# wdecoster/inquiSTR

Measured on AMD Instinct MI355X. Metric: loci/sec genotyped (inquiSTR call hot path, device-resident batch = L0), higher is better.
Workload: dtype u32/i64; 1 GPU; unphased100k: 100000 loci/GPU x 30 reads x ~200 CIGAR ops, --unphased, device-resident SoA (L0); loci_per_gpu=100000, pairs_per_gpu=3000000, cigar_ops_per_gpu=600007253, minlen=5, support=3, total_loci=100000

## Files before the change

inquistr_amd/csrc/cigar_walk.h:

```cpp
#pragma once
#include <type_traits>

#include "wave_primitives.h"

namespace inq {

typedef unsigned int u32x4 __attribute__((ext_vector_type(4)));

constexpr uint32_t ST_INDEX = 1u, ST_CIGAR_OP = 2u, ST_RANGE = 4u, ST_PHASE = 8u, ST_LOCUS = 16u, ST_HINT = 32u, ST_AUX = 64u,
                   ST_INTERNAL = 128u;

constexpr uint32_t PM_CLIP = 1u, PM_FETCHED = 2u, PM_KEPT = 4u;
constexpr int PM_GRP_SHIFT = 4;
constexpr uint32_t PM_CHOSEN = 64u;

constexpr uint32_t RB_UNMAPPED = 1u, RB_REVERSE = 2u, RB_HAS_HP = 4u, RB_IS_2D = 8u, RB_SA_PANIC = 16u;

constexpr int kQueueCap = 128;

struct Window {
    uint32_t se;
    uint32_t ee;
    uint32_t se1;
    uint32_t width;
    uint32_t minlen;
};

__device__ __forceinline__ Window make_window(uint32_t start, uint32_t end, uint32_t minlen) {
    Window W;
    W.se = start - 10u;
    W.ee = end + 10u;
    W.se1 = W.se + 1u;
    W.width = W.ee >= W.se1 ? W.ee - W.se1 : 0u;
    W.minlen = minlen;
    return W;
}

struct BatchView {
    const uint4 *cigar4;
    const uint4 *reads;
    const uint32_t *pair_read;
    uint64_t n_reads;
    uint64_t n_cigar4;
};

struct QueueEntry {
    u32x4 w;
    uint2 info;
    uint2 pad;
};
struct WaveLds {
    QueueEntry q[kQueueCap];
    unsigned long long acc[64];
    unsigned int flags[64];
    unsigned int endc[64];
};

static_assert(sizeof(WaveLds) == 5120, "a larger WaveLds costs resident workgroups per CU");
static_assert(kQueueCap >= 128, "the list takes the spare words of 128 queue entries");
__device__ __forceinline__ void cont_put(WaveLds &L, uint32_t i, uint32_t cur4, uint32_t rw, uint32_t carry) {
    L.q[i].pad = make_uint2(cur4, rw);
    L.q[64u + i].pad.x = carry;
}
__device__ __forceinline__ void cont_get(const WaveLds &L, int i, uint32_t &cur4, uint32_t &rw, uint32_t &carry) {
    const uint2 r = L.q[i].pad;
    cur4 = r.x, rw = r.y;
    carry = L.q[64 + i].pad.x;
}

struct PairMeta {
    uint32_t off4, nc, pos, misc;
};

__device__ __forceinline__ PairMeta load_pair_meta(const BatchView &b, uint64_t first, int cnt, int lane,
                                                    uint32_t &status, bool &valid) {
    PairMeta m{0u, 0u, 0u, 0u};
    valid = false;
    if (lane < cnt) {
        uint32_t ri = b.pair_read[first + (uint64_t)lane];
        if ((uint64_t)ri < b.n_reads) {
            uint4 r = b.reads[ri];
            uint64_t n4 = ((uint64_t)r.y + 3u) >> 2;
            if (r.y < 0x10000000u && (uint64_t)r.x + n4 <= b.n_cigar4) {
                m.off4 = r.x;
                m.nc = r.y | ((r.w & (RB_IS_2D << 8)) ? 0x80000000u : 0u);
                m.pos = r.z;
                m.misc = r.w;
                valid = true;
            } else {
                status |= ST_INDEX;
            }
        } else {
            status |= ST_INDEX;
        }
    }
    return m;
}

__device__ __forceinline__ uint32_t meta_stage_a(const BatchView &b, uint64_t first, int cnt, int lane) {
    return lane < cnt ? b.pair_read[first + (uint64_t)lane] : 0xffffffffu;
}
__device__ __forceinline__ uint4 meta_stage_b(const BatchView &b, uint32_t ri) {
    return (uint64_t)ri < b.n_reads ? b.reads[ri] : make_uint4(0u, 0xffffffffu, 0u, 0u);
}
__device__ __forceinline__ PairMeta meta_stage_c(const BatchView &b, const uint4 r, int cnt, int lane, uint32_t &status,
                                                  bool &valid) {
    PairMeta m{0u, 0u, 0u, 0u};
    valid = false;
    if (lane < cnt) {
        const uint64_t n4 = ((uint64_t)r.y + 3u) >> 2;
        if (r.y < 0x10000000u && (uint64_t)r.x + n4 <= b.n_cigar4) {
            m.off4 = r.x;
            m.nc = r.y | ((r.w & (RB_IS_2D << 8)) ? 0x80000000u : 0u);
            m.pos = r.z;
            m.misc = r.w;
            valid = true;
        } else {
            status |= ST_INDEX;
        }
    }
    return m;
}

constexpr uint32_t kConsume = 0x18Du;

__device__ __forceinline__ uint32_t ref_advance(uint32_t op, uint32_t len) {
    return len & (uint32_t)__builtin_amdgcn_sbfe((int)kConsume, op, 1u);
}
constexpr uint32_t kConsume32 = kConsume | (kConsume << 16);
__device__ __forceinline__ uint32_t ref_advance_raw(uint32_t w) {
    return (w >> 4) & (uint32_t)__builtin_amdgcn_sbfe((int)kConsume32, w, 1u);
}
constexpr uint32_t kBadOp32 = 0xFE00FE00u;
__device__ __forceinline__ uint32_t bad_ops(const u32x4 w) {
    return (kBadOp32 >> (w.x & 31u)) | (kBadOp32 >> (w.y & 31u)) | (kBadOp32 >> (w.z & 31u)) | (kBadOp32 >> (w.w & 31u));
}
__device__ __forceinline__ void advance4(const u32x4 w, uint32_t &e1, uint32_t &e2, uint32_t &e3, uint32_t &tot) {
    e1 = ref_advance_raw(w.x), e2 = e1 + ref_advance_raw(w.y);
    e3 = e2 + ref_advance_raw(w.z), tot = e3 + ref_advance_raw(w.w);
}

__device__ __forceinline__ void drain_queue(WaveLds &L, uint32_t &qcount, const Window &W, int lane) {
    __builtin_amdgcn_wave_barrier();
    for (uint32_t base = 0; base < qcount; base += 64u) {
        const uint32_t e = base + (uint32_t)lane;
        if (e < qcount) {
            const u32x4 w = L.q[e].w;
            const uint2 info = L.q[e].info;
            const uint32_t rel = info.x;
            const uint32_t slot = info.y & 63u;
            const uint32_t cand_mask = (info.y & 64u) ? 0x06u : 0x16u;
            const uint32_t op0 = w.x & 15u, op1 = w.y & 15u, op2 = w.z & 15u, op3 = w.w & 15u;
            const uint32_t l0 = w.x >> 4, l1 = w.y >> 4, l2 = w.z >> 4, l3 = w.w >> 4;
            const uint32_t e1 = ref_advance(op0, l0), e2 = e1 + ref_advance(op1, l1), e3 = e2 + ref_advance(op2, l2);
            int32_t s = 0;
            uint32_t clip = 0;
#define INQ_OP(op, len, ee_)                                                                              \
    {                                                                                                     \
        const bool hit = ((cand_mask >> (op)) & 1u) && (len) > W.minlen && (rel + (ee_)) < W.width;        \
        const int32_t v = ((op) == 2u) ? -(int32_t)(len) : (int32_t)(len);                                \
        s += hit ? v : 0;                                                                                 \
        clip |= (hit && (op) == 4u) ? 1u : 0u;                                                            \
    }
            INQ_OP(op0, l0, 0u)
            INQ_OP(op1, l1, e1)
            INQ_OP(op2, l2, e2)
            INQ_OP(op3, l3, e3)
#undef INQ_OP
            if (s != 0) atomicAdd(&L.acc[slot], (unsigned long long)(long long)s);
            if (clip) atomicOr(&L.flags[slot], 1u);
        }
    }
    qcount = 0;
    __builtin_amdgcn_wave_barrier();
}

__device__ __forceinline__ bool push_window_lanes(WaveLds &L, uint32_t &qcount, bool inw, const u32x4 w, uint32_t x,
                                                  uint32_t tot, uint32_t info, uint32_t info_mask) {
    const uint64_t mask = ballot64(inw);
    if (mask) {
        QueueEntry *const tail = &L.q[qcount];
        if (inw) {
            const uint32_t idx = __builtin_amdgcn_mbcnt_hi((uint32_t)(mask >> 32), __builtin_amdgcn_mbcnt_lo((uint32_t)mask, 0u));
            tail[idx].w = w;
            tail[idx].info = make_uint2(x - tot, info & info_mask);
        }
        qcount += (uint32_t)__popcll(mask);
    }
    return mask != 0ull && qcount > 64u;
}

template <bool UNPHASED>
__device__ __forceinline__ void read_epilogue(const PairMeta &m, bool valid, int cnt, const Window &W, int lane,
                                              uint32_t end_carry, uint32_t &status, WaveLds &L, int64_t &val,
                                              uint32_t &meta) {
    val = 0;
    meta = 0;
    if (lane < cnt && valid) {
        const uint32_t pos = m.pos;
        const uint32_t mapq = m.misc & 0xffu, bits = (m.misc >> 8) & 0xffu, phase = (m.misc >> 16) & 0xffu;
        uint32_t rlen = end_carry - (pos + 1u);
        if ((bits & RB_UNMAPPED) || rlen == 0u) rlen = 1u;
        const uint32_t rend = pos + rlen;
        const bool fetched = ((int32_t)pos < 0 || pos < W.ee) && rend > W.se;
        bool skip;
        if (UNPHASED)
            skip = W.se < pos || rend < W.ee || mapq <= 10u;
        else
            skip = !(bits & RB_HAS_HP) || (W.se < pos && rend < W.ee) || mapq <= 10u;
        const bool kept = fetched && !skip;
        uint32_t grp = 0u;
        bool bad_phase = false;
        if (!UNPHASED && kept) {
            if (phase > 2u)
                bad_phase = true;
            else
                grp = phase;
        }
        if (bad_phase) status |= ST_PHASE;
        if (kept && (bits & RB_SA_PANIC)) status |= ST_AUX;
        val = (int64_t)L.acc[lane];
        meta = ((L.flags[lane] & 1u) ? PM_CLIP : 0u) | (fetched ? PM_FETCHED : 0u) | (kept ? PM_KEPT : 0u) |
               (grp << PM_GRP_SHIFT);
    }
}

template <bool UNPHASED, int AUX>
__device__ __forceinline__ void walk_pairs_whole(const BatchView &b, const PairMeta &m, bool valid, int cnt,
                                           const Window &W, int lane, uint32_t &status, WaveLds &L, int64_t &val,
                                           uint32_t &meta) {
    L.acc[lane] = 0ull;
    L.flags[lane] = 0u;
    uint32_t qcount = 0;
    uint32_t lane_range = 0, lane_bad = 0;
    uint32_t end_carry = 0;

    const uint4 *cigar4 = b.cigar4;
    asm volatile("" : "+s"(cigar4));
    int hk = 0;
    uint32_t hc = 0, h_nchunks = 1, h_off4 = 0, h_n4 = 0;
    auto head_load = [&]() {
        if (hk < cnt) {
            h_off4 = readlane_u32(m.off4, hk);
            const uint32_t nc = readlane_u32(m.nc, hk) & 0x7fffffffu;
            h_n4 = (nc + 3u) >> 2;
            h_nchunks = max(1u, (nc + 255u) >> 8);
        } else {
            h_off4 = 0;
            h_n4 = 0;
            h_nchunks = 1;
        }
    };
    auto issue = [&]() -> u32x4 {
        const __amdgpu_buffer_rsrc_t rsrc =
            __builtin_amdgcn_make_buffer_rsrc((void *)(cigar4 + h_off4), (short)0, (int)(h_n4 * 16u), 0x00020000);
        const u32x4 v = __builtin_amdgcn_raw_buffer_load_b128(rsrc, (int)((hc * 64u + (uint32_t)lane) * 16u), 0, AUX);
        ++hc;
        if (hc >= h_nchunks) {
            ++hk;
            hc = 0;
            head_load();
        }
        return v;
    };
    head_load();
    u32x4 qa = issue(), qb = issue(), qc = issue(), qd = issue();

    int tk = 0;
    uint32_t tc = 0, t_nchunks = 1, t_nc = 0, t_info = 0, carry = 0;
    auto tail_load = [&]() {
        if (tk < cnt) {
            const uint32_t ncp = readlane_u32(m.nc, tk);
            t_nc = ncp & 0x7fffffffu;
            t_nchunks = max(1u, (t_nc + 255u) >> 8);
            carry = readlane_u32(m.pos, tk) + 1u;
            t_info = (uint32_t)tk | ((ncp >> 31) << 6);
            lane_range |= carry;
        }
    };
    tail_load();

    auto step = [&](const u32x4 w) {
        uint32_t e1, e2, e3, tot;
        advance4(w, e1, e2, e3, tot);
        const uint32_t incl = wave_inclusive_scan_u32(tot);
        lane_bad |= bad_ops(w);
        lane_range |= carry + incl;
        const uint32_t x = (carry - W.se1) + incl;
        if (push_window_lanes(L, qcount, x < W.width + tot, w, x, tot, t_info, ~0u)) drain_queue(L, qcount, W, lane);
        carry += readlane_u32(incl, 63);
        ++tc;
        if (tc >= t_nchunks) {
            end_carry = writelane_u32(end_carry, carry, tk);
            ++tk;
            tc = 0;
            tail_load();
        }
    };

    while (tk < cnt) {
        step(qa);
        qa = issue();
        if (tk < cnt) step(qb);
        qb = issue();
        if (tk < cnt) step(qc);
        qc = issue();
        if (tk < cnt) step(qd);
        qd = issue();
    }
    if (qcount) drain_queue(L, qcount, W, lane);
    if (ballot64((lane_bad & 1u) != 0u)) status |= ST_CIGAR_OP;
    if (ballot64((lane_range >> 31) != 0u)) status |= ST_RANGE;

    read_epilogue<UNPHASED>(m, valid, cnt, W, lane, end_carry, status, L, val, meta);
}

constexpr uint32_t RP_CHECKED = 1u;


constexpr int kHeadLanes = 8;
constexpr int kHeadLines = 4;
__device__ __forceinline__ void head_row_scan_u32(uint32_t x, bool upper, uint32_t &incl, uint32_t &tot) {
    const uint32_t s = row_inclusive_scan_u32(x);
    const uint32_t lower = (uint32_t)__builtin_amdgcn_ds_swizzle((int)s, 0x10 | (0x07 << 5));
    incl = s - (upper ? lower : 0u);
    tot = (uint32_t)__builtin_amdgcn_ds_swizzle((int)incl, 0x18 | (0x07 << 5));
}

struct RowStream {
    uint32_t cur4;
    uint32_t carry;
    uint32_t st;
};
constexpr uint32_t RS_STOP = 128u, RS_LIVE = 256u;
constexpr int RS_LEFT = 9;
constexpr uint32_t kLineMask = 7u;
constexpr uint32_t kRowMaxGroups = 1u << (32 - RS_LEFT);
__host__ __device__ constexpr uint32_t cigar_groups(uint32_t nc) { return (nc + 3u) >> 2; }
static_assert(cigar_groups((1u << 25) - 4u) == kRowMaxGroups - 1u && cigar_groups((1u << 25) - 3u) == kRowMaxGroups,
              "the longest read the row walk takes is 2^25 - 4 ops");
constexpr int RW_SLOT = 23, RW_2D = 30, RW_PROMISED = 31;
static_assert((kRowMaxGroups - 1u) >> RW_SLOT == 0u && (63u << RW_SLOT) >> RW_2D == 0u, "the fields of the row word lie apart");
__device__ __forceinline__ uint32_t rw_pack(uint32_t groups, uint32_t is_2d, bool promised) {
    return groups | (is_2d << RW_2D) | (promised ? 1u << RW_PROMISED : 0u);
}
__device__ __forceinline__ uint32_t rw_groups(uint32_t rw) { return rw & (kRowMaxGroups - 1u); }
__device__ __forceinline__ uint32_t rw_groups_slot0(uint32_t rw) { return rw & ((1u << RW_2D) - 1u); }
__device__ __forceinline__ uint32_t rw_slot(uint32_t rw) { return (rw >> RW_SLOT) & 63u; }
__device__ __forceinline__ uint32_t rw_2d(uint32_t rw) { return (rw >> RW_2D) & 1u; }
__device__ __forceinline__ bool rw_promised(uint32_t rw) { return (rw >> RW_PROMISED) != 0u; }
__device__ __forceinline__ uint32_t row_state(uint32_t groups, uint32_t slot, uint32_t is_2d, bool promised) {
    return (groups << RS_LEFT) | slot | (is_2d << 6) | (promised ? RS_STOP : 0u) | RS_LIVE;
}

template <bool UNPHASED, int AUX>
__device__ __forceinline__ void walk_pairs_rows(const BatchView &b, const PairMeta &m, bool valid, int cnt,
                                                const Window &W, int lane, bool checks, uint32_t &status, WaveLds &L,
                                                int64_t &val, uint32_t &meta) {
    L.acc[lane] = 0ull;
    L.flags[lane] = 0u;
    L.endc[lane] = m.pos + 1u;
    uint32_t qcount = 0;
    uint32_t lane_err = ((m.pos + 1u) >> 31) << 1;
    const uint64_t row_heads = 0x0001000100010001ull;
    const __amdgpu_buffer_rsrc_t rsrc =
        __builtin_amdgcn_make_buffer_rsrc((void *)b.cigar4, (short)0, (int)(uint32_t)(b.n_cigar4 * 16u), 0x00020000);

    const uint32_t d_w = rw_pack(cigar_groups(m.nc & 0x0fffffffu), m.nc >> 31, ((m.misc >> 24) & RP_CHECKED) != 0u);

    const int rl = lane & (kRowLanes - 1);
    const int hl = lane & (kHeadLanes - 1);
    const int hrow = lane >> 3;
    const bool upper = (lane & kHeadLanes) != 0;

    auto issue = [&](const RowStream &S) -> u32x4 {
        const uint32_t g = (S.cur4 & ~kLineMask) + (uint32_t)rl;
        const bool on = g - S.cur4 < (S.st >> RS_LEFT);
        return __builtin_amdgcn_raw_buffer_load_b128(rsrc, (int)(on ? g * 16u : 0xfffffff0u), 0, AUX);
    };
    auto head_issue = [&](const RowStream &S) -> u32x4 {
        return __builtin_amdgcn_raw_buffer_load_b128(rsrc, (int)((uint32_t)hl < (S.st >> RS_LEFT) ? S.cur4 : 0xfffffff0u), 0, AUX);
    };
    auto step = [&](const u32x4 w, RowStream &S, auto lanes, bool last) {
        constexpr uint32_t LANES = decltype(lanes)::value;
        const bool live = S.st != 0u;
        uint32_t e1, e2, e3, tot, incl, rtot;
        advance4(w, e1, e2, e3, tot);
        if (LANES == (uint32_t)kHeadLanes) {
            head_row_scan_u32(tot, upper, incl, rtot);
        } else {
            incl = row_inclusive_scan_u32(tot);
            rtot = row_last(incl);
        }
        if (checks) {
            if (live) {
                lane_err |= bad_ops(w) & 1u;
                lane_err |= ((S.carry + incl) >> 31) << 1;
            }
        }
        const uint32_t x = (S.carry - W.se1) + incl;
        if (push_window_lanes(L, qcount, live && x < W.width + tot, w, x, tot, S.st, 127u)) drain_queue(L, qcount, W, lane);
        S.carry += rtot;
        if (LANES == (uint32_t)kHeadLanes) {
            S.cur4 += 16u * LANES;
            const bool done = last || (S.st >> RS_LEFT) <= LANES || ((S.st & RS_STOP) && S.carry > W.ee);
            if (live && done && hl == 0) L.endc[S.st & 63u] = S.carry;
            S.st = done ? 0u : S.st - (LANES << RS_LEFT);
        } else {
            const uint32_t end4 = (S.cur4 & ~kLineMask) + LANES;
            const uint32_t lim = end4 - S.cur4;
            S.cur4 = end4;
            if (live) {
                if ((S.st >> RS_LEFT) <= lim || ((S.st & RS_STOP) && S.carry > W.ee)) {
                    if (rl == 0) L.endc[S.st & 63u] = S.carry;
                    S.st = 0u;
                } else {
                    S.st -= lim << RS_LEFT;
                }
            }
        }
    };
    using Head = std::integral_constant<uint32_t, (uint32_t)kHeadLanes>;
    using Later = std::integral_constant<uint32_t, (uint32_t)kRowLanes>;

    L.q[lane].pad = make_uint2(m.off4, d_w);
    __builtin_amdgcn_wave_barrier();
    auto assign = [&](RowStream &S, int k0) -> u32x4 {
        S.st = 0u;
        uint32_t voff = 0xfffffff0u;
        if (k0 < cnt) {
            const uint2 d = L.q[k0 + hrow].pad;
            const uint32_t r_w = d.y, skip = d.x & kLineMask;
            S.cur4 = ((d.x & ~kLineMask) + (uint32_t)hl) * 16u;
            S.carry = L.endc[k0 + hrow];
            if (rw_groups_slot0(r_w) != 0u && !(rw_promised(r_w) && S.carry > W.ee)) {
                const uint32_t left = min(rw_groups_slot0(r_w) + skip, (uint32_t)((kHeadLines + 1) * kHeadLanes));
                S.st = row_state(left, (uint32_t)(k0 + hrow), rw_2d(r_w), rw_promised(r_w));
                if ((uint32_t)hl - skip < left - skip) voff = S.cur4;
            }
        }
        return __builtin_amdgcn_raw_buffer_load_b128(rsrc, (int)voff, 0, AUX);
    };
    RowStream sa{0u, 0u, 0u}, sb = sa, sc = sa, sd = sa;
    u32x4 qa, qb, qc, qd;
    for (int k0 = 0; k0 < cnt; k0 += 4 * kHeadLanes) {
        qa = assign(sa, k0);
        qb = assign(sb, k0 + kHeadLanes);
        qc = assign(sc, k0 + 2 * kHeadLanes);
        qd = assign(sd, k0 + 3 * kHeadLanes);
        if (ballot64((sa.st | sb.st | sc.st | sd.st) != 0u)) {
            int line = 0;
            do {
                const bool last = ++line == kHeadLines;
                if (ballot64(sa.st != 0u)) step(qa, sa, Head{}, last);
                qa = head_issue(sa);
                if (ballot64(sb.st != 0u)) step(qb, sb, Head{}, last);
                qb = head_issue(sb);
                if (ballot64(sc.st != 0u)) step(qc, sc, Head{}, last);
                qc = head_issue(sc);
                if (ballot64(sd.st != 0u)) step(qd, sd, Head{}, last);
                qd = head_issue(sd);
            } while (ballot64((sa.st | sb.st | sc.st | sd.st) != 0u));
        }
    }

    __builtin_amdgcn_wave_barrier();
    const uint32_t endc0 = L.endc[lane];
    const uint2 own = L.q[lane].pad;
    const uint32_t groups = rw_groups_slot0(own.y) & (kRowMaxGroups - 1u);
    const bool promised = rw_promised(own.y);
    const uint32_t head_groups = (uint32_t)(kHeadLines * kHeadLanes) - (own.x & kLineMask);
    const bool cont = groups > head_groups && !(promised && endc0 > W.ee);
    const uint64_t cmask = ballot64(cont);
    if (cmask) {
        const int ncont = (int)__popcll(cmask);
        if (cont) {
            const uint32_t i = __builtin_amdgcn_mbcnt_hi((uint32_t)(cmask >> 32), __builtin_amdgcn_mbcnt_lo((uint32_t)cmask, 0u));
            cont_put(L, i, own.x + head_groups, (own.y - head_groups) | ((uint32_t)lane << RW_SLOT), endc0);
        }
        __builtin_amdgcn_wave_barrier();

        int next = 0;
        auto claim = [&](RowStream &S) {
            if (next >= ncont) return;
            const bool idle = S.st == 0u;
            const uint64_t need = ballot64(idle) & row_heads;
            if (need == 0ull) return;
            const int below = (int)__builtin_amdgcn_mbcnt_hi((uint32_t)(need >> 32), __builtin_amdgcn_mbcnt_lo((uint32_t)need, 0u));
            const int k = next + below - ((idle && rl != 0) ? 1 : 0);
            next += (int)__popcll(need);
            if (idle && k < ncont) {
                uint32_t r_w;
                cont_get(L, k, S.cur4, r_w, S.carry);
                S.st = row_state(rw_groups(r_w), rw_slot(r_w), rw_2d(r_w), rw_promised(r_w));
            }
        };
        sa.st = sb.st = sc.st = sd.st = 0u;
        claim(sa);
        qa = issue(sa);
        claim(sb);
        qb = issue(sb);
        claim(sc);
        qc = issue(sc);
        claim(sd);
        qd = issue(sd);
        while (ballot64((sa.st | sb.st | sc.st | sd.st) != 0u)) {
            if (ballot64(sa.st != 0u)) {
                step(qa, sa, Later{}, false);
                claim(sa);
            }
            qa = issue(sa);
            if (ballot64(sb.st != 0u)) {
                step(qb, sb, Later{}, false);
                claim(sb);
            }
            qb = issue(sb);
            if (ballot64(sc.st != 0u)) {
                step(qc, sc, Later{}, false);
                claim(sc);
            }
            qc = issue(sc);
            if (ballot64(sd.st != 0u)) {
                step(qd, sd, Later{}, false);
                claim(sd);
            }
            qd = issue(sd);
        }
    }
    if (qcount) drain_queue(L, qcount, W, lane);
    if (ballot64((lane_err & 1u) != 0u)) status |= ST_CIGAR_OP;
    if (ballot64((lane_err & 2u) != 0u)) status |= ST_RANGE;
    __builtin_amdgcn_wave_barrier();
    read_epilogue<UNPHASED>(m, valid, cnt, W, lane, L.endc[lane], status, L, val, meta);
}

template <bool UNPHASED, int AUX>
__device__ __forceinline__ void walk_pairs(const BatchView &b, const PairMeta &m, bool valid, int cnt,
                                           const Window &W, int lane, uint32_t &status, WaveLds &L, int64_t &val,
                                           uint32_t &meta) {
    const bool checked = lane < cnt && valid && ((m.misc >> 24) & RP_CHECKED) != 0u;
    const bool too_long = lane < cnt && valid && cigar_groups(m.nc & 0x0fffffffu) >= kRowMaxGroups;
    if (ballot64(checked) != 0ull && ballot64(too_long) == 0ull && W.ee >= W.se1 && b.n_cigar4 < (1ull << 28)) {
        const bool checks = ballot64(lane < cnt && valid && !checked) != 0ull;
        walk_pairs_rows<UNPHASED, AUX>(b, m, valid, cnt, W, lane, checks, status, L, val, meta);
    } else {
        walk_pairs_whole<UNPHASED, AUX>(b, m, valid, cnt, W, lane, status, L, val, meta);
    }
}

}
```

Before: 509.3 million loci/s.

## Precompute head row states, specialize checks, and drain queue one wave at a time

Row state and starting carry for each read are now computed once per lane and stored in LDS, so the head assignment only loads them. This removes the per-assign recomputation of groups, skip and the promise check. The head-loop state no longer counts down, and the done/issue tests compare against per-line thresholds instead. The head loop is also instantiated twice on whether checks are on, which removes a runtime branch from every step. The ballot of live lanes is reused for the window push, and drain_queue now handles only the newest 64 entries instead of emptying the whole queue, which shortens each drain but makes drains more frequent and adds code size.

```diff
diff --git a/inquistr_amd/csrc/cigar_walk.h b/inquistr_amd/csrc/cigar_walk.h
--- a/inquistr_amd/csrc/cigar_walk.h
+++ b/inquistr_amd/csrc/cigar_walk.h
@@ -142,7 +142,8 @@
 
 __device__ __forceinline__ void drain_queue(WaveLds &L, uint32_t &qcount, const Window &W, int lane) {
     __builtin_amdgcn_wave_barrier();
-    for (uint32_t base = 0; base < qcount; base += 64u) {
+    const uint32_t base = qcount > 64u ? qcount - 64u : 0u;
+    {
         const uint32_t e = base + (uint32_t)lane;
         if (e < qcount) {
             const u32x4 w = L.q[e].w;
@@ -171,13 +172,12 @@
             if (clip) atomicOr(&L.flags[slot], 1u);
         }
     }
-    qcount = 0;
+    qcount = base;
     __builtin_amdgcn_wave_barrier();
 }
 
-__device__ __forceinline__ bool push_window_lanes(WaveLds &L, uint32_t &qcount, bool inw, const u32x4 w, uint32_t x,
-                                                  uint32_t tot, uint32_t info, uint32_t info_mask) {
-    const uint64_t mask = ballot64(inw);
+__device__ __forceinline__ bool push_window_lanes(WaveLds &L, uint32_t &qcount, uint64_t mask, bool inw, const u32x4 w,
+                                                  uint32_t x, uint32_t tot, uint32_t info, uint32_t info_mask) {
     if (mask) {
         QueueEntry *const tail = &L.q[qcount];
         if (inw) {
@@ -287,7 +287,8 @@
         lane_bad |= bad_ops(w);
         lane_range |= carry + incl;
         const uint32_t x = (carry - W.se1) + incl;
-        if (push_window_lanes(L, qcount, x < W.width + tot, w, x, tot, t_info, ~0u)) drain_queue(L, qcount, W, lane);
+        const bool inw = x < W.width + tot;
+        if (push_window_lanes(L, qcount, ballot64(inw), inw, w, x, tot, t_info, ~0u)) drain_queue(L, qcount, W, lane);
         carry += readlane_u32(incl, 63);
         ++tc;
         if (tc >= t_nchunks) {
@@ -345,7 +346,7 @@
     return groups | (is_2d << RW_2D) | (promised ? 1u << RW_PROMISED : 0u);
 }
 __device__ __forceinline__ uint32_t rw_groups(uint32_t rw) { return rw & (kRowMaxGroups - 1u); }
-__device__ __forceinline__ uint32_t rw_groups_slot0(uint32_t rw) { return rw & ((1u << RW_2D) - 1u); }
+__device__ __forceinline__ uint32_t line_word(uint32_t off4) { return ((off4 & ~kLineMask) << 4) | (off4 & kLineMask); }
 __device__ __forceinline__ uint32_t rw_slot(uint32_t rw) { return (rw >> RW_SLOT) & 63u; }
 __device__ __forceinline__ uint32_t rw_2d(uint32_t rw) { return (rw >> RW_2D) & 1u; }
 __device__ __forceinline__ bool rw_promised(uint32_t rw) { return (rw >> RW_PROMISED) != 0u; }
@@ -378,11 +379,12 @@
         const bool on = g - S.cur4 < (S.st >> RS_LEFT);
         return __builtin_amdgcn_raw_buffer_load_b128(rsrc, (int)(on ? g * 16u : 0xfffffff0u), 0, AUX);
     };
-    auto head_issue = [&](const RowStream &S) -> u32x4 {
-        return __builtin_amdgcn_raw_buffer_load_b128(rsrc, (int)((uint32_t)hl < (S.st >> RS_LEFT) ? S.cur4 : 0xfffffff0u), 0, AUX);
-    };
-    auto step = [&](const u32x4 w, RowStream &S, auto lanes, bool last) {
+    auto head_issue = [&](const RowStream &S, uint32_t next_thr) -> u32x4 {
+        return __builtin_amdgcn_raw_buffer_load_b128(rsrc, (int)(S.st >= next_thr ? S.cur4 : 0xfffffff0u), 0, AUX);
+    };
+    auto step = [&](const u32x4 w, RowStream &S, uint64_t live_mask, auto lanes, auto ck, bool last, uint32_t done_thr) {
         constexpr uint32_t LANES = decltype(lanes)::value;
+        constexpr int CK = decltype(ck)::value;
         const bool live = S.st != 0u;
         uint32_t e1, e2, e3, tot, incl, rtot;
         advance4(w, e1, e2, e3, tot);
@@ -392,26 +394,30 @@
             incl = row_inclusive_scan_u32(tot);
             rtot = row_last(incl);
         }
-        if (checks) {
+        if (CK == 2 ? checks : CK == 1) {
             if (live) {
                 lane_err |= bad_ops(w) & 1u;
                 lane_err |= ((S.carry + incl) >> 31) << 1;
             }
         }
         const uint32_t x = (S.carry - W.se1) + incl;
-        if (push_window_lanes(L, qcount, live && x < W.width + tot, w, x, tot, S.st, 127u)) drain_queue(L, qcount, W, lane);
+        const bool in = x < W.width + tot;
+        uint64_t in_mask = ballot64(in);
+        asm("" : "+s"(in_mask));
+        if (push_window_lanes(L, qcount, in_mask & live_mask, live && in, w, x, tot, S.st, 127u)) drain_queue(L, qcount, W, lane);
         S.carry += rtot;
+        const bool past = CK == 0 ? S.carry > W.ee : (S.st & RS_STOP) && S.carry > W.ee;
         if (LANES == (uint32_t)kHeadLanes) {
             S.cur4 += 16u * LANES;
-            const bool done = last || (S.st >> RS_LEFT) <= LANES || ((S.st & RS_STOP) && S.carry > W.ee);
+            const bool done = last || S.st < done_thr || past;
             if (live && done && hl == 0) L.endc[S.st & 63u] = S.carry;
-            S.st = done ? 0u : S.st - (LANES << RS_LEFT);
+            S.st = done ? 0u : S.st;
         } else {
             const uint32_t end4 = (S.cur4 & ~kLineMask) + LANES;
             const uint32_t lim = end4 - S.cur4;
             S.cur4 = end4;
             if (live) {
-                if ((S.st >> RS_LEFT) <= lim || ((S.st & RS_STOP) && S.carry > W.ee)) {
+                if ((S.st >> RS_LEFT) <= lim || past) {
                     if (rl == 0) L.endc[S.st & 63u] = S.carry;
                     S.st = 0u;
                 } else {
@@ -422,52 +428,67 @@
     };
     using Head = std::integral_constant<uint32_t, (uint32_t)kHeadLanes>;
     using Later = std::integral_constant<uint32_t, (uint32_t)kRowLanes>;
-
-    L.q[lane].pad = make_uint2(m.off4, d_w);
+    using AsChecks = std::integral_constant<int, 2>;
+
+    {
+        const uint32_t groups = cigar_groups(m.nc & 0x0fffffffu), skip = m.off4 & kLineMask;
+        const bool nothing = groups == 0u || (rw_promised(d_w) && m.pos + 1u > W.ee);
+        const uint32_t left = min(groups + skip, (uint32_t)((kHeadLines + 1) * kHeadLanes));
+        const uint32_t st = nothing ? 0u : row_state(left, (uint32_t)lane, m.nc >> 31, rw_promised(d_w));
+        L.q[lane].pad = make_uint2(line_word(m.off4), d_w);
+        L.q[64 + lane].pad = make_uint2(st, m.pos + 1u);
+    }
     __builtin_amdgcn_wave_barrier();
+    const uint32_t hl16 = (uint32_t)hl * 16u;
     auto assign = [&](RowStream &S, int k0) -> u32x4 {
         S.st = 0u;
         uint32_t voff = 0xfffffff0u;
         if (k0 < cnt) {
-            const uint2 d = L.q[k0 + hrow].pad;
-            const uint32_t r_w = d.y, skip = d.x & kLineMask;
-            S.cur4 = ((d.x & ~kLineMask) + (uint32_t)hl) * 16u;
-            S.carry = L.endc[k0 + hrow];
-            if (rw_groups_slot0(r_w) != 0u && !(rw_promised(r_w) && S.carry > W.ee)) {
-                const uint32_t left = min(rw_groups_slot0(r_w) + skip, (uint32_t)((kHeadLines + 1) * kHeadLanes));
-                S.st = row_state(left, (uint32_t)(k0 + hrow), rw_2d(r_w), rw_promised(r_w));
-                if ((uint32_t)hl - skip < left - skip) voff = S.cur4;
-            }
+            const uint2 d = L.q[64 + k0 + hrow].pad;
+            const uint32_t lw = L.q[k0 + hrow].pad.x;
+            S.st = d.x, S.carry = d.y;
+            S.cur4 = (lw & ~(16u * kLineMask + 15u)) | hl16;
+            if ((uint32_t)hl >= (lw & kLineMask) && (uint32_t)hl < (S.st >> RS_LEFT)) voff = S.cur4;
         }
         return __builtin_amdgcn_raw_buffer_load_b128(rsrc, (int)voff, 0, AUX);
     };
     RowStream sa{0u, 0u, 0u}, sb = sa, sc = sa, sd = sa;
     u32x4 qa, qb, qc, qd;
-    for (int k0 = 0; k0 < cnt; k0 += 4 * kHeadLanes) {
-        qa = assign(sa, k0);
-        qb = assign(sb, k0 + kHeadLanes);
-        qc = assign(sc, k0 + 2 * kHeadLanes);
-        qd = assign(sd, k0 + 3 * kHeadLanes);
-        if (ballot64((sa.st | sb.st | sc.st | sd.st) != 0u)) {
-            int line = 0;
-            do {
-                const bool last = ++line == kHeadLines;
-                if (ballot64(sa.st != 0u)) step(qa, sa, Head{}, last);
-                qa = head_issue(sa);
-                if (ballot64(sb.st != 0u)) step(qb, sb, Head{}, last);
-                qb = head_issue(sb);
-                if (ballot64(sc.st != 0u)) step(qc, sc, Head{}, last);
-                qc = head_issue(sc);
-                if (ballot64(sd.st != 0u)) step(qd, sd, Head{}, last);
-                qd = head_issue(sd);
-            } while (ballot64((sa.st | sb.st | sc.st | sd.st) != 0u));
-        }
-    }
+    auto head = [&](auto ck) {
+        for (int k0 = 0; k0 < cnt; k0 += 4 * kHeadLanes) {
+            qa = assign(sa, k0);
+            qb = assign(sb, k0 + kHeadLanes);
+            qc = assign(sc, k0 + 2 * kHeadLanes);
+            qd = assign(sd, k0 + 3 * kHeadLanes);
+            if (ballot64((sa.st | sb.st | sc.st | sd.st) != 0u)) {
+                uint32_t line = 0;
+                do {
+                    const bool last = ++line == (uint32_t)kHeadLines;
+                    const uint32_t done_thr = (line * kHeadLanes + 1u) << RS_LEFT;
+                    uint32_t next_thr = ((uint32_t)hl + line * kHeadLanes + 1u) << RS_LEFT;
+                    asm("" : "+v"(next_thr));
+                    uint64_t lm;
+                    if ((lm = ballot64(sa.st != 0u))) step(qa, sa, lm, Head{}, ck, last, done_thr);
+                    qa = head_issue(sa, next_thr);
+                    if ((lm = ballot64(sb.st != 0u))) step(qb, sb, lm, Head{}, ck, last, done_thr);
+                    qb = head_issue(sb, next_thr);
+                    if ((lm = ballot64(sc.st != 0u))) step(qc, sc, lm, Head{}, ck, last, done_thr);
+                    qc = head_issue(sc, next_thr);
+                    if ((lm = ballot64(sd.st != 0u))) step(qd, sd, lm, Head{}, ck, last, done_thr);
+                    qd = head_issue(sd, next_thr);
+                } while (ballot64((sa.st | sb.st | sc.st | sd.st) != 0u));
+            }
+        }
+    };
+    if (checks)
+        head(std::integral_constant<int, 1>{});
+    else
+        head(std::integral_constant<int, 0>{});
 
     __builtin_amdgcn_wave_barrier();
     const uint32_t endc0 = L.endc[lane];
     const uint2 own = L.q[lane].pad;
-    const uint32_t groups = rw_groups_slot0(own.y) & (kRowMaxGroups - 1u);
+    const uint32_t groups = rw_groups(own.y);
     const bool promised = rw_promised(own.y);
     const uint32_t head_groups = (uint32_t)(kHeadLines * kHeadLanes) - (own.x & kLineMask);
     const bool cont = groups > head_groups && !(promised && endc0 > W.ee);
@@ -476,7 +497,7 @@
         const int ncont = (int)__popcll(cmask);
         if (cont) {
             const uint32_t i = __builtin_amdgcn_mbcnt_hi((uint32_t)(cmask >> 32), __builtin_amdgcn_mbcnt_lo((uint32_t)cmask, 0u));
-            cont_put(L, i, own.x + head_groups, (own.y - head_groups) | ((uint32_t)lane << RW_SLOT), endc0);
+            cont_put(L, i, (own.x >> 4) + (uint32_t)(kHeadLines * kHeadLanes), (own.y - head_groups) | ((uint32_t)lane << RW_SLOT), endc0);
         }
         __builtin_amdgcn_wave_barrier();
 
@@ -505,23 +526,23 @@
         claim(sd);
         qd = issue(sd);
         while (ballot64((sa.st | sb.st | sc.st | sd.st) != 0u)) {
-            if (ballot64(sa.st != 0u)) {
-                step(qa, sa, Later{}, false);
+            if (const uint64_t lm = ballot64(sa.st != 0u)) {
+                step(qa, sa, lm, Later{}, AsChecks{}, false, 0u);
                 claim(sa);
             }
             qa = issue(sa);
-            if (ballot64(sb.st != 0u)) {
-                step(qb, sb, Later{}, false);
+            if (const uint64_t lm = ballot64(sb.st != 0u)) {
+                step(qb, sb, lm, Later{}, AsChecks{}, false, 0u);
                 claim(sb);
             }
             qb = issue(sb);
-            if (ballot64(sc.st != 0u)) {
-                step(qc, sc, Later{}, false);
+            if (const uint64_t lm = ballot64(sc.st != 0u)) {
+                step(qc, sc, lm, Later{}, AsChecks{}, false, 0u);
                 claim(sc);
             }
             qc = issue(sc);
-            if (ballot64(sd.st != 0u)) {
-                step(qd, sd, Later{}, false);
+            if (const uint64_t lm = ballot64(sd.st != 0u)) {
+                step(qd, sd, lm, Later{}, AsChecks{}, false, 0u);
                 claim(sd);
             }
             qd = issue(sd);
```

Result: faster. 524.7 million loci/s (median of 6 runs) (+3.0%).
